# Advaith-Sajeev/LiDAR-Vision-VQA

Measured on AMD Instinct MI355X. Metric: fused tokens/sec/GPU + cross-attn MFMA-roofline % (32k pts x 196 patches), higher is better.
Workload: dtype bf16; 1 GPU; BASELINE configs[1]: 32768-pt scenes (Dist-C) -> hard voxelise (0.1, 0.1, 0.2) T=10 max=60000 + MeanVFE; pillars (0.2, 0.2, 8.0) T=20 max=30000 -> PillarVFE[64] -> PointPillarScatter 512x512 (as an index map; sparse key stream: K|V computed only for the cells with a pillar in their 3x3 neighbourhood, by LayerNorm and the K|V projection folded onto the 64-channel conv token, every other key from th; parallelism=scene-parallel x1

## Files before the change

### include/lvq.h

```cpp
#ifndef LVQ_H
#define LVQ_H

#include <stddef.h>
#include <stdint.h>

#ifdef __cplusplus
extern "C" {
#endif

typedef void *lvq_stream_t;
typedef uint16_t lvq_bf16;

enum {
    LVQ_OK = 0,
    LVQ_EINVAL = -1,
    LVQ_EWORKSPACE = -2,
    LVQ_ELAUNCH = -3,
    LVQ_EOVERFLOW = -4,
    LVQ_EUNSUPPORTED = -5
};

const char *lvq_version(void);
const char *lvq_strerror(int code);

typedef struct lvq_tuning {
    int32_t attn_no32;
    int32_t attn32_nw;
    int32_t attn_pipe;
    int32_t attn_nsplit;
    int32_t attn_qt;
    int32_t attn_nw;
    int32_t gemm_no_gemv;
    int32_t gemm_stream_c_mb;
    int32_t gemm_no256;
    int32_t gemm_no256x256;
    int32_t gemm_256x256_min_tiles;
    int32_t gemm_ln_tiles;
    int32_t pillar_vfe_generic;
    int32_t voxel_path;
    int32_t pairs_one_wg;
    int32_t ca_fused_variant;
    uint64_t ca_fused_stamps;
    int32_t reserved[8];
} lvq_tuning;
void lvq_tuning_defaults(lvq_tuning *t);
int lvq_set_tuning(const lvq_tuning *t);
int lvq_get_tuning(lvq_tuning *t);


int lvq_mask_points_by_range(const float *pts, int64_t n, int c, const float *range_host, uint8_t *keep,
                             lvq_stream_t stream);

size_t lvq_voxelize_hard_workspace_bytes(int64_t n_points, int n_scenes);
int lvq_voxelize_hard(const float *pts, const int32_t *scene_off, int64_t n_points, int n_scenes, int c,
                      const float *range_host, const float *vsize_host, const int32_t *grid_host,
                      int max_pts, int max_voxels, int break_on_cap, int64_t voxel_capacity,
                      float *voxels, int32_t *coords_bzyx, int32_t *num_pts, int32_t *scene_voxel_off,
                      void *ws, size_t ws_bytes, lvq_stream_t stream);

int lvq_voxelize_mean(const float *pts, const int32_t *scene_off, int64_t n_points, int n_scenes, int c,
                      const float *range_host, const float *vsize_host, const int32_t *grid_host, int max_pts,
                      int max_voxels, int64_t voxel_capacity, float *voxel_features, int32_t *coords_bzyx,
                      int32_t *num_pts, int32_t *scene_voxel_off, void *ws, size_t ws_bytes, lvq_stream_t stream);

int lvq_mean_vfe(const float *voxels, const int32_t *num_pts, int64_t m_cap, const int32_t *n_voxels_dev,
                 int t, int c, float *out, lvq_stream_t stream);

int lvq_pillar_vfe(const float *voxels, const int32_t *num_pts, const int32_t *coords_bzyx, int64_t m_cap,
                   const int32_t *n_voxels_dev, int t, int c, int n_layers, const float *const *w_host,
                   const float *const *scale_host, const float *const *shift_host, const int32_t *cin_host,
                   const int32_t *cout_host, int flags, const float *vsize_host, const float *offset_host,
                   float *out, lvq_stream_t stream);

size_t lvq_voxelize_dynamic_workspace_bytes(int64_t n_points, int batch_size, const int32_t *grid_host, int ndim);
int lvq_voxelize_dynamic(const float *pts, int64_t n, int c, int batch_size, const float *range_host,
                         const float *vsize_host, const int32_t *grid_host, int ndim, int32_t *unq_inv,
// ... 215 lines not shown
```

### lidar-vision-vqa_amd/_ffi.py

```python
from __future__ import annotations

import ctypes
import os
import re
from typing import List, Optional, Sequence

import torch

_HERE = os.path.dirname(os.path.abspath(__file__))
LIB_PATH = os.environ.get("LVQ_LIB_PATH") or os.path.join(_HERE, "liblvq_hip.so")
HEADER_PATH = os.path.join(os.path.dirname(_HERE), "include", "lvq.h")

LVQ_OK = 0
LVQ_EUNSUPPORTED = -5


class LvqError(RuntimeError):
    pass


_lib: Optional[ctypes.CDLL] = None


class Tuning(ctypes.Structure):
    _fields_ = [(n, ctypes.c_int32) for n in (
        "attn_no32", "attn32_nw", "attn_pipe", "attn_nsplit", "attn_qt", "attn_nw", "gemm_no_gemv", "gemm_stream_c_mb", "gemm_no256",
        "gemm_no256x256", "gemm_256x256_min_tiles", "gemm_ln_tiles", "pillar_vfe_generic", "voxel_path", "pairs_one_wg",
        "ca_fused_variant")] + [("ca_fused_stamps", ctypes.c_uint64), ("reserved", ctypes.c_int32 * 8)]


TUNING_FIELDS = tuple(n for n, _ in Tuning._fields_ if n != "reserved")


def tuning_from_env(env=None) -> dict:
    e = os.environ if env is None else env

    def flag(name):
        return 1 if e.get(name) else 0

    def num(name):
        return int(e[name]) if e.get(name) else 0

    return {
        "attn_no32": flag("LVQ_ATTN_NO32"), "attn32_nw": num("LVQ_ATTN32_NW"),
        "attn_pipe": -1 if e.get("LVQ_ATTN_NO_PIPE") else flag("LVQ_ATTN_PIPE"),
        "attn_nsplit": num("LVQ_ATTN_NSPLIT"), "attn_qt": num("LVQ_ATTN_QT"), "attn_nw": num("LVQ_ATTN_NW"),
        "gemm_no_gemv": flag("LVQ_GEMM_NO_GEMV"),
        "gemm_stream_c_mb": -1 if e.get("LVQ_GEMM_NO_STREAM_C") else num("LVQ_GEMM_STREAM_C_MB"),
        "gemm_no256": flag("LVQ_GEMM_NO256"), "gemm_no256x256": flag("LVQ_GEMM_NO256X256"),
        "gemm_256x256_min_tiles": num("LVQ_GEMM_256X256_MIN_TILES"), "gemm_ln_tiles": flag("LVQ_GEMM_LN_TILES"),
        "pillar_vfe_generic": flag("LVQ_PILLAR_VFE_GENERIC"),
        "voxel_path": 2 if e.get("LVQ_VOXEL_LEGACY") else flag("LVQ_VOXEL_BINNED"),
        "pairs_one_wg": flag("LVQ_PAIRS_ONE_WG"), "ca_fused_variant": num("LVQ_CA_DBG"), "ca_fused_stamps": 0,
    }


def set_tuning(**fields) -> dict:
    rec = tuning_from_env()
    for k, v in fields.items():
        if k not in TUNING_FIELDS:
            raise LvqError(f"lvq_tuning has no field {k!r}")
        rec[k] = int(v)
    t = Tuning()
    for k, v in rec.items():
        setattr(t, k, v)
    check(lib().lvq_set_tuning(ctypes.byref(t)), "lvq_set_tuning")
    return rec


def get_tuning() -> dict:
    t = Tuning()
    check(lib().lvq_get_tuning(ctypes.byref(t)), "lvq_get_tuning")
    return {k: int(getattr(t, k)) for k in TUNING_FIELDS}


class tuning:

    def __init__(self, **fields):
        self.fields = fields

    def __enter__(self):
        self.old = get_tuning()
        cur = dict(self.old)
        cur.update({k: int(v) for k, v in self.fields.items()})
        _push(cur)
        return self
# ... 87 lines not shown
```

### lidar-vision-vqa_amd/csrc/bev_tiles.hip

```cpp
#include "common.h"
#include <type_traits>
#include <utility>

namespace bt {

typedef __attribute__((ext_vector_type(8))) short bf16x8;
typedef __attribute__((ext_vector_type(4))) float f32x4;
typedef __attribute__((ext_vector_type(2))) __bf16 bf16x2_t;
typedef uint32_t u32x4 __attribute__((ext_vector_type(4)));

__device__ __forceinline__ uint32_t pack_bf16(float a, float b) {
    bf16x2_t p = {(__bf16)a, (__bf16)b};
    return *reinterpret_cast<uint32_t *>(&p);
}
typedef _Float16 f16x2_t __attribute__((ext_vector_type(2)));
__device__ __forceinline__ uint32_t pack_f16(float a, float b) {
    f16x2_t p = {(_Float16)a, (_Float16)b};
    return __builtin_bit_cast(uint32_t, p);
}

constexpr int TS = 8, TCELLS = 64;
constexpr int NPIECE = 8, PCELLS = 8;
constexpr int PH = 4, PW = 6, PHALO = PH * PW;
constexpr int NSLOT = NPIECE * PHALO;
// ... 782 lines not shown
            };
            f32x4 te_a[2 * JH], te_b[2 * JH];
            int2 pd_a, pd_b;
            request(0, te_a, pd_a);
            if (has_nx) conv_tile(ih_nx, buf ^ 1);
            request(1, te_b, pd_b);
            emit(0, te_a, pd_a);
            request(2, te_a, pd_a);
            emit(1, te_b, pd_b);
            request(3, te_b, pd_b);
            emit(2, te_a, pd_a);
            emit(3, te_b, pd_b);
        }
        buf ^= 1;
    }
}

struct ConvArgs {
    const float *feat;
    const int32_t *idx;
    const int32_t *live_list;
    const int2 *piece_dirty;
    const int32_t *counts;
    const float *w9, *b9;
    const uint16_t *rh, *rl;
    const float *r0;
    float c0, inv_d, eps;
    int S, H, W;
    uint16_t *th, *tl;
    float *rstd;
    int32_t *key;
};

template <bool X3>
__global__ void __launch_bounds__(512) k_conv_rows(ConvArgs a) {
    constexpr int C = 64, NWV = 8;
    extern __shared__ __attribute__((aligned(16))) uint8_t smem[];
    uint16_t *t_hi = reinterpret_cast<uint16_t *>(smem);
    uint16_t *t_lo = t_hi + 2 * TCELLS * C;
    float *halo = reinterpret_cast<float *>(t_lo + 2 * TCELLS * C);
    int32_t *idxh = reinterpret_cast<int32_t *>(halo + NSLOT * C);
    float *part = reinterpret_cast<float *>(idxh + 2 * 256);
    float *w9s = part + 2 * 4 * TCELLS;
    float *b9s = w9s + 9 * C;
    float *r0s = b9s + C;
    uint16_t *r_hi = reinterpret_cast<uint16_t *>(r0s + C);
    uint16_t *r_lo = r_hi + C * C;
    const int tid = threadIdx.x, lane = tid & 63, wid = tid >> 6, l15 = lane & 15, g4 = lane >> 4;
    const int tw = a.W / TS;
    const int n_live = a.counts[0];
    const int64_t n_groups = ((int64_t)n_live + NPIECE - 1) / NPIECE;
    const int64_t g_begin = blockIdx.x, g_end = n_groups, g_step = gridDim.x;

    for (int e = tid; e < 9 * C; e += 512) w9s[e] = a.w9[(e % C) * 9 + e / C];
    if (tid < C) { b9s[tid] = a.b9 ? a.b9[tid] : 0.f; r0s[tid] = a.r0[tid]; }
    for (int e = tid; e < C * C / 8; e += 512) {
        reinterpret_cast<u32x4 *>(r_hi)[e] = reinterpret_cast<const u32x4 *>(a.rh)[e];
        if (X3) reinterpret_cast<u32x4 *>(r_lo)[e] = reinterpret_cast<const u32x4 *>(a.rl)[e];
    }
    auto load_idx = [&](int64_t g, int &code_out) -> int {
        code_out = -1;
        if (tid >= NSLOT) return -1;
        const int j = tid / PHALO, hc = tid - j * PHALO;
        const int64_t k = g * NPIECE + j;
        if (k >= n_live) return -1;
        const int code = a.live_list[k];
        code_out = code;
        const int p = code & 7, ts = code >> 3, t = ts / a.S, sc = ts - t * a.S;
        int y0, x0;
        piece_origin(t, p, tw, y0, x0);
        const int gy = y0 - 1 + hc / PW, gx = x0 - 1 + hc % PW;
        return (gy >= 0 && gy < a.H && gx >= 0 && gx < a.W) ? a.idx[((int64_t)sc * a.H + gy) * a.W + gx] : -1;
    };
    auto store_idx = [&](int32_t *ih, int v, int code) {
        if (tid < NSLOT) {
            ih[tid] = v;
            if (tid % PHALO == 0) ih[200 + tid / PHALO] = code;
        }
    };
    auto dma_halo = [&](const int32_t *ih) {
        for (int q = wid; q < NSLOT / 4; q += NWV) {
            const int slot = q * 4 + (lane >> 4);
            const int row = ih[slot];
            if (row >= 0)
                __builtin_amdgcn_global_load_lds((const __attribute__((address_space(1))) void *)(a.feat + (int64_t)row * C + 4 * l15),
                                                 (__attribute__((address_space(3))) void *)(halo + q * 4 * C), 16, 0, 0);
        }
    };
    auto conv_tile = [&](const int32_t *ih, int buf, int64_t g) {
        const int cell = tid >> 3, cg = (tid & 7) * 8, hb = (cell >> 3) * PHALO, cy = (cell >> 2) & 1, cx = cell & 3;
        float acc[8];
#pragma unroll
        for (int c = 0; c < 8; ++c) acc[c] = b9s[cg + c];
#pragma unroll
        for (int rr = 0; rr < 3; ++rr)
#pragma unroll
            for (int k = 0; k < 3; ++k) {
                const int slot = hb + (cy + rr) * PW + cx + k;
                if (ih[slot] >= 0) {
                    const f32x4 v0 = *reinterpret_cast<const f32x4 *>(halo + slot * C + cg), v1 = *reinterpret_cast<const f32x4 *>(halo + slot * C + cg + 4);
                    const f32x4 k0 = *reinterpret_cast<const f32x4 *>(w9s + (rr * 3 + k) * C + cg), k1 = *reinterpret_cast<const f32x4 *>(w9s + (rr * 3 + k) * C + cg + 4);
#pragma unroll
                    for (int c = 0; c < 4; ++c) { acc[c] = fmaf(v0[c], k0[c], acc[c]); acc[4 + c] = fmaf(v1[c], k1[c], acc[4 + c]); }
                }
            }
        uint32_t hi[4], lo[4];
#pragma unroll
        for (int c = 0; c < 4; ++c) {
            const float y0 = gelu_erf(acc[2 * c]), y1 = gelu_erf(acc[2 * c + 1]);
            hi[c] = pack_bf16(y0, y1);
            lo[c] = pack_bf16(y0 - __uint_as_float(hi[c] << 16), y1 - __uint_as_float(hi[c] & 0xffff0000u));
        }
        const int ch = (tid & 7) ^ ((cell >> 1) & 7);
        *reinterpret_cast<u32x4 *>(t_hi + (buf * TCELLS + cell) * C + ch * 8) = u32x4{hi[0], hi[1], hi[2], hi[3]};
        if (X3) *reinterpret_cast<u32x4 *>(t_lo + (buf * TCELLS + cell) * C + ch * 8) = u32x4{lo[0], lo[1], lo[2], lo[3]};
        const int code = ih[200 + (cell >> 3)];
        if (code >= 0) {
            const int2 pd = a.piece_dirty[g * NPIECE + (cell >> 3)];
            if ((pd.y >> (cell & 7)) & 1) {
                const int64_t orow = pd.x + __popc((unsigned)pd.y & ((1u << (cell & 7)) - 1u));
                *reinterpret_cast<u32x4 *>(a.th + orow * C + cg) = u32x4{hi[0], hi[1], hi[2], hi[3]};
                if (X3) *reinterpret_cast<u32x4 *>(a.tl + orow * C + cg) = u32x4{lo[0], lo[1], lo[2], lo[3]};
            }
        }
    };
    auto load_t = [&](int buf, int gq, bf16x8 &th0, bf16x8 &th1, bf16x8 &tl0, bf16x8 &tl1) {
        const int row = gq * 16 + l15;
        const int c0 = (g4 ^ ((row >> 1) & 7)) * 8, c1 = ((4 + g4) ^ ((row >> 1) & 7)) * 8;
        th0 = *reinterpret_cast<const bf16x8 *>(t_hi + (buf * TCELLS + row) * C + c0);
        th1 = *reinterpret_cast<const bf16x8 *>(t_hi + (buf * TCELLS + row) * C + c1);
        if (X3) {
            tl0 = *reinterpret_cast<const bf16x8 *>(t_lo + (buf * TCELLS + row) * C + c0);
            tl1 = *reinterpret_cast<const bf16x8 *>(t_lo + (buf * TCELLS + row) * C + c1);
        }
    };

    if (tid < 256) { idxh[tid] = -1; idxh[256 + tid] = -1; }
    __syncthreads();
    if (g_begin >= g_end) return;
    {
        int c0, c1;
        const int i0 = load_idx(g_begin, c0);
        const int i1 = g_begin + g_step < g_end ? load_idx(g_begin + g_step, c1) : (c1 = -1, -1);
        store_idx(idxh, i0, c0);
        store_idx(idxh + 256, i1, c1);
    }
    __syncthreads();
    dma_halo(idxh);
    asm volatile("s_waitcnt vmcnt(0)" ::: "memory");
    __syncthreads();
    conv_tile(idxh, 0, g_begin);
    int buf = 0;
    for (int64_t g = g_begin, it = 0; g < g_end; g += g_step, ++it) {
        __syncthreads();
        const int32_t *ih_cur = idxh + (it & 1) * 256, *ih_nx = idxh + ((it + 1) & 1) * 256;
        const bool has_nx = g + g_step < g_end, has_n2 = g + 2 * g_step < g_end;
        if (has_nx) dma_halo(ih_nx);
        const int my_code = tid < TCELLS ? ih_cur[200 + (tid >> 3)] : -1;
        int c2 = -1;
        const int i2 = has_n2 ? load_idx(g + 2 * g_step, c2) : -1;
        {
            const int rt = wid & 3;
            const uint16_t *rp = r_hi + (16 * rt + l15) * C + 8 * g4, *rpl = r_lo + (16 * rt + l15) * C + 8 * g4;
            const bf16x8 ra0 = *reinterpret_cast<const bf16x8 *>(rp), ra1 = *reinterpret_cast<const bf16x8 *>(rp + 32);
            bf16x8 rl0 = ra0, rl1 = ra1;
            if (X3) { rl0 = *reinterpret_cast<const bf16x8 *>(rpl); rl1 = *reinterpret_cast<const bf16x8 *>(rpl + 32); }
            const f32x4 rinit = *reinterpret_cast<const f32x4 *>(r0s + 16 * rt + 4 * g4);
#pragma unroll
            for (int u = 0; u < 2; ++u) {
                const int gq = 2 * (wid >> 2) + u;
                bf16x8 th0, th1, tl0, tl1;
                load_t(buf, gq, th0, th1, tl0, tl1);
                f32x4 v = rinit;
                v = __builtin_amdgcn_mfma_f32_16x16x32_bf16(ra0, th0, v, 0, 0, 0);
                v = __builtin_amdgcn_mfma_f32_16x16x32_bf16(ra1, th1, v, 0, 0, 0);
                if (X3) {
                    v = __builtin_amdgcn_mfma_f32_16x16x32_bf16(ra0, tl0, v, 0, 0, 0);
                    v = __builtin_amdgcn_mfma_f32_16x16x32_bf16(ra1, tl1, v, 0, 0, 0);
                    v = __builtin_amdgcn_mfma_f32_16x16x32_bf16(rl0, th0, v, 0, 0, 0);
                    v = __builtin_amdgcn_mfma_f32_16x16x32_bf16(rl1, th1, v, 0, 0, 0);
                }
                float sq = (v[0] * v[0] + v[1] * v[1]) + (v[2] * v[2] + v[3] * v[3]);
                sq += __shfl_xor(sq, 16);
                sq += __shfl_xor(sq, 32);
                if (g4 == 0) part[(buf * 4 + rt) * TCELLS + gq * 16 + l15] = sq;
            }
        }
        asm volatile("s_waitcnt vmcnt(0)" ::: "memory");
        __syncthreads();
        store_idx(idxh + (it & 1) * 256, i2, c2);
        if (tid < TCELLS && my_code >= 0) {
            const int cell = tid;
            const int2 pd = a.piece_dirty[g * NPIECE + (cell >> 3)];
            if ((pd.y >> (cell & 7)) & 1) {
                const int64_t orow = pd.x + __popc((unsigned)pd.y & ((1u << (cell & 7)) - 1u));
                const float *pr = part + buf * 4 * TCELLS;
                const float ss = (pr[cell] + pr[TCELLS + cell]) + (pr[2 * TCELLS + cell] + pr[3 * TCELLS + cell]) + a.c0;
                a.rstd[orow] = 1.0f / sqrtf(ss * a.inv_d + a.eps);
                a.key[orow] = ((my_code >> 3) / a.S) * TCELLS + (my_code & 7) * PCELLS + (cell & 7);
            }
        }
        if (has_nx) conv_tile(ih_nx, buf ^ 1, g + g_step);
        buf ^= 1;
    }
}

struct KvRowArgs {
    const uint16_t *th, *tl;
    const float *rstd;
    const int32_t *key;
    const int32_t *n_rows;
    const uint16_t *mh, *ml;
    const float *m0;
    const float *te;
    uint16_t *out;
    int k_fp16;
};

template <int N> __device__ __forceinline__ void vm_wait() { asm volatile("s_waitcnt vmcnt(%0)" ::"n"(N) : "memory"); }
template <int OFF> __device__ __forceinline__ void vm_load16(f32x4 &d, const void *p) {
    asm volatile("global_load_dwordx4 %0, %1, off offset:%2" : "=&v"(d) : "v"(p), "n"(OFF) : "memory");
}
template <class T> __device__ __forceinline__ void vm_load4(T &d, const void *p) {
    static_assert(sizeof(T) == 4, "one dword");
    asm volatile("global_load_dword %0, %1, off" : "=&v"(d) : "v"(p) : "memory");
}
__device__ __forceinline__ void vm_dma16(const void *src, uint32_t dst) {
    uint32_t keep;
    asm volatile("s_mov_b32 %0, m0\n\ts_mov_b32 m0, %2\n\ts_nop 0\n\tglobal_load_lds_dwordx4 %1, off\n\ts_mov_b32 m0, %0"
                 : "=&s"(keep) : "v"(src), "s"(dst) : "memory");
}
template <class T> __device__ __forceinline__ void landed(T &x) { asm volatile("" : "+v"(x)); }
template <int... I, class F> __device__ __forceinline__ void static_for(std::integer_sequence<int, I...>, F &&f) { (f(std::integral_constant<int, I>{}), ...); }
template <int N, class F> __device__ __forceinline__ void static_for(F &&f) { static_for(std::make_integer_sequence<int, N>{}, f); }

template <int J, bool X3, bool TH>
__global__ void __launch_bounds__(512) k_kv_rows(KvRowArgs a) {
    constexpr int N = 128 * J, C = 64, JH = J / 2;
    static_assert(J % 2 == 0, "even J");
    extern __shared__ __attribute__((aligned(16))) uint8_t smem[];
    uint16_t *t_hi = reinterpret_cast<uint16_t *>(smem);
    uint16_t *t_lo = t_hi + 2 * TCELLS * C;
    float *pbias = reinterpret_cast<float *>(t_lo + 2 * TCELLS * C);
    constexpr int SROW = N + 8;
    uint16_t *sbuf = reinterpret_cast<uint16_t *>(pbias + N);
    const int tid = threadIdx.x, lane = tid & 63, wid = tid >> 6, l15 = lane & 15, g4 = lane >> 4;
    const int64_t n_rows = *a.n_rows;
    const int64_t n_groups = (n_rows + TCELLS - 1) / TCELLS;
    const bool x8 = gridDim.x >= 16 && gridDim.x % 16 == 0;
    const int nxcd = x8 ? 8 : 1;
    const int xcd = x8 ? (int)blockIdx.x & 7 : 0;
    const int half = x8 ? ((int)blockIdx.x >> 3) & 1 : (int)blockIdx.x & 1;
    const int wg_r = x8 ? (int)blockIdx.x >> 4 : (int)blockIdx.x >> 1, wg_R = x8 ? (int)gridDim.x >> 4 : ((int)gridDim.x + 1) >> 1;
    const int64_t per_x = (n_groups + nxcd - 1) / nxcd;
    const int64_t x_begin = (int64_t)xcd * per_x, x_end = x_begin + per_x < n_groups ? x_begin + per_x : n_groups;
    const int64_t g_begin = x_begin + wg_r, g_end = x_end, g_step = wg_R;
    const int ncol0 = half * N;
    const bool as_f16 = a.k_fp16 != 0 && half == 0;
    for (int e = tid; e < N; e += 512) pbias[e] = a.m0[ncol0 + e];

    bf16x8 wf[J][2], wfl[X3 ? J : 1][2];
#pragma unroll
    for (int j = 0; j < J; ++j) {
        const int n = ncol0 + 16 * J * wid + (TH ? 32 * (j >> 1) + 8 * (l15 >> 2) + 4 * (j & 1) + (l15 & 3) : 16 * j + l15);
        wf[j][0] = *reinterpret_cast<const bf16x8 *>(a.mh + (int64_t)n * C + 8 * g4);
        wf[j][1] = *reinterpret_cast<const bf16x8 *>(a.mh + (int64_t)n * C + 32 + 8 * g4);
        if (X3) {
// ... 233 lines not shown
}

extern "C" int lvq_bev_tile_kv(const float *pillar_feat, const int32_t *idx_map, const int32_t *live_list, const int32_t *piece_dirty,
                               const int32_t *counts, int64_t cap_tiles, int batch, int ny, int nx, int c_in, const float *w9, const float *b9,
                               const lvq_bf16 *m, const lvq_bf16 *m_lo, const float *m0, const lvq_bf16 *r, const lvq_bf16 *r_lo, const float *r0,
                               float c0, int d_ln, float eps, const void *t_tiled, int t_f16, int n, int k_fp16, lvq_bf16 *kv, void *ws,
                               size_t ws_bytes, lvq_stream_t stream) {
    if (batch <= 0 || ny <= 0 || nx <= 0 || cap_tiles <= 0 || d_ln <= 0 || !idx_map || !live_list || !piece_dirty || !counts || !w9 || !m || !m0 || !r ||
        !r0 || !t_tiled || !kv)
        return LVQ_EINVAL;
    if ((m_lo == nullptr) != (r_lo == nullptr)) return LVQ_EINVAL;
    if ((k_fp16 || t_f16) && ws == nullptr) return LVQ_EUNSUPPORTED;
    if (c_in != 64 || (ny % 8) || (nx % 8) || (n % 256) || n < 256 || n > 1024) return LVQ_EUNSUPPORTED;
    if (((uintptr_t)pillar_feat | (uintptr_t)m | (uintptr_t)m_lo | (uintptr_t)r | (uintptr_t)r_lo | (uintptr_t)m0 | (uintptr_t)r0 | (uintptr_t)t_tiled |
         (uintptr_t)kv) & 15)
        return LVQ_EUNSUPPORTED;
    bt::KvArgs a;
    a.feat = pillar_feat; a.idx = idx_map; a.live_list = live_list; a.piece_dirty = reinterpret_cast<const int2 *>(piece_dirty); a.counts = counts;
    a.w9 = w9; a.b9 = b9; a.mh = m; a.ml = m_lo; a.m0 = m0; a.rh = r; a.rl = r_lo; a.r0 = r0; a.c0 = c0; a.inv_d = 1.0f / (float)d_ln; a.eps = eps;
    a.te = static_cast<const float *>(t_tiled); a.S = batch; a.H = ny; a.W = nx; a.out = kv;
    hipStream_t st = lvq_s(stream);
    const bool x3 = m_lo != nullptr;
    if (ws != nullptr) {
        LvqArena arena(ws, ws_bytes);
        uint16_t *th = arena.take<uint16_t>((size_t)cap_tiles * 64 * 64);
        uint16_t *tl = arena.take<uint16_t>((size_t)cap_tiles * 64 * 64);
        float *rstd = arena.take<float>((size_t)cap_tiles * 64);
        int32_t *key = arena.take<int32_t>((size_t)cap_tiles * 64);
        if (!arena.ok) return LVQ_EWORKSPACE;
        bt::ConvArgs c;
        c.feat = pillar_feat; c.idx = idx_map; c.live_list = live_list; c.piece_dirty = a.piece_dirty; c.counts = counts; c.w9 = w9; c.b9 = b9;
        c.rh = r; c.rl = r_lo; c.r0 = r0; c.c0 = c0; c.inv_d = a.inv_d; c.eps = eps; c.S = batch; c.H = ny; c.W = nx;
        c.th = th; c.tl = x3 ? tl : nullptr; c.rstd = rstd; c.key = key;
        const size_t lds = (size_t)2 * 2 * bt::TCELLS * 64 * 2 + (size_t)bt::NSLOT * 64 * 4 + 2 * 256 * 4 + (size_t)2 * 4 * bt::TCELLS * 4 + 9 * 64 * 4 +
                           64 * 4 + 64 * 4 + (size_t)2 * 64 * 64 * 2;
        static LvqLdsOnce once;
        if (!lvq_ensure_lds(once, {(const void *)bt::k_conv_rows<false>, (const void *)bt::k_conv_rows<true>}, lds)) return LVQ_ELAUNCH;
        int64_t grid = (int64_t)lvq_cu_count();
        if (grid > cap_tiles) grid = cap_tiles;
        if (x3) hipLaunchKernelGGL((bt::k_conv_rows<true>), dim3((unsigned)grid), dim3(512), lds, st, c);
        else    hipLaunchKernelGGL((bt::k_conv_rows<false>), dim3((unsigned)grid), dim3(512), lds, st, c);
        bt::KvRowArgs k;
        k.th = th; k.tl = x3 ? tl : nullptr; k.rstd = rstd; k.key = key; k.n_rows = counts + 2; k.mh = m; k.ml = m_lo; k.m0 = m0; k.te = static_cast<const float *>(t_tiled); k.out = kv; k.k_fp16 = k_fp16;
        switch (n / 128) {
            case 2: return launch_kv_rows<2>(k, x3, t_f16 != 0, cap_tiles, st);
            case 4: return launch_kv_rows<4>(k, x3, t_f16 != 0, cap_tiles, st);
            case 6: return launch_kv_rows<6>(k, x3, t_f16 != 0, cap_tiles, st);
            case 8: return launch_kv_rows<8>(k, x3, t_f16 != 0, cap_tiles, st);
            default: return LVQ_EUNSUPPORTED;
        }
    }
    switch (n / 128) {
        case 2: return launch_tile_kv<2>(a, x3, cap_tiles, st);
        case 4: return launch_tile_kv<4>(a, x3, cap_tiles, st);
        case 6: return launch_tile_kv<6>(a, x3, cap_tiles, st);
        case 8: return launch_tile_kv<8>(a, x3, cap_tiles, st);
        default: return LVQ_EUNSUPPORTED;
    }
}

extern "C" int lvq_bev_scene_pairs(const int32_t *row_src, int batch, int n_tiles, int row_base, int cap_tiles, int32_t *pair_src,
                                   int32_t *pair_info, lvq_stream_t stream) {
    if (!row_src || !pair_src || !pair_info || batch <= 0 || n_tiles <= 0 || cap_tiles <= 0 || row_base < 0) return LVQ_EINVAL;
    if (((uintptr_t)row_src & 15) || (int64_t)n_tiles * bt::TCELLS > 0x7fffffff || batch > 65535) return LVQ_EUNSUPPORTED;
    if (cap_tiles >= n_tiles && cap_tiles >= 2 && !lvq_tune().pairs_one_wg) {
        const int64_t ne = (int64_t)n_tiles * bt::TCELLS;
        int64_t chunk = (ne + 63) / 64;
        chunk = (chunk + 1023) / 1024 * 1024;
        const int nch = (int)((ne + chunk - 1) / chunk);
        hipLaunchKernelGGL(bt::k_scene_pair_count, dim3(nch, batch), dim3(bt::PAIR2_NT), 0, lvq_s(stream), row_src, n_tiles, row_base, cap_tiles, (int)chunk,
                           pair_src);
        hipLaunchKernelGGL(bt::k_scene_pair_write, dim3(nch, batch), dim3(bt::PAIR2_NT), 0, lvq_s(stream), row_src, n_tiles, row_base, cap_tiles, (int)chunk,
// ... 47 lines not shown
```

### lidar-vision-vqa_amd/fusion.py

```python
from __future__ import annotations

import math
import os
from typing import Dict, List, Optional, Tuple

import torch
import torch.nn as nn

from . import _ffi as F
from . import autograd_route as AG
from . import ops
from .ops import BF

NUM_VIEWS = 6
CAM_VIEWS = ("CAM_FRONT", "CAM_FRONT_RIGHT", "CAM_FRONT_LEFT", "CAM_BACK", "CAM_BACK_RIGHT", "CAM_BACK_LEFT")


class _HipModule(nn.Module):

    def __init__(self):
        super().__init__()
        object.__setattr__(self, "_wcache", {})
        self.precision: Optional[str] = None

# ... 362 lines not shown
        ver = tuple((p.data_ptr(), p._version) for p in params) + (self._mode(), fused, k16, bool(os.environ.get("LVQ_KV_ONE_LAUNCH")),
                                                                   bool(os.environ.get("LVQ_KV_T_FP16")))
        key = ("kv_buffer", H, W, dev)
        hw, d = H * W, self.d_model
        rows = hw + batch * hw
        hit = self._pe_cache.get(key)
        if hit is not None and hit[0] == ver:
            if hit[1][0].shape[0] >= rows:
                return hit[1]
            bufs = []
            for old in hit[1]:
                buf = torch.empty((rows, 2 * d), dtype=torch.bfloat16, device=dev)
                buf[:hw].copy_(old[:hw])
                bufs.append(buf)
            self._pe_cache[key] = (ver, bufs)
            return bufs
        self._pe_cache.pop(("signed_totals", H, W, dev), None)
        idx = torch.full((1, H, W), -1, dtype=torch.int32, device=dev)
        live, dirty, src, counts = ops.bev_tiles(idx, 1, H, W, dev, 0, force_all=True)
        feat = torch.zeros((1, C), dtype=torch.float32, device=dev)
        x = None if fused else self._tile_tokens(feat, idx, live, dirty, counts, hw, 1, H, W)
        bufs = []
        for li, blk in enumerate(self.blocks):
            blk.precision = self.precision
            buf = torch.empty((rows, 2 * d), dtype=torch.bfloat16, device=dev)
            if fused:
                self._tile_kv(li, feat, idx, live, dirty, counts, hw, 1, H, W, buf[:hw], k_fp16=k16 and li == 0)
            else:
                ops.linear_live_rows(x, blk._w(blk.ca.in_proj_weight), blk.ca.in_proj_bias, counts[2:], (d, 3 * d), out=buf[:hw])
            bufs.append(buf)
        self._pe_cache[key] = (ver, bufs)
        return bufs

    def _q16_ok(self, blk: "VATBlock", qp: BF) -> bool:
        params = [self.query, self.view_embed, blk.sa_ln.weight, blk.sa_ln.bias, blk.sa.in_proj_weight, blk.sa.in_proj_bias, blk.sa.out_proj.weight,
                  blk.sa.out_proj.bias, blk.ca_ln.weight, blk.ca_ln.bias, blk.ca.in_proj_weight, blk.ca.in_proj_bias]
        ver = tuple((p.data_ptr(), p._version) for p in params) + (self._mode(),)
        hit = self._pe_cache.get("q16_ok")
        if hit is not None and hit[0] == ver:
            return hit[1]
        dh = blk.d_model // blk.n_heads
        qmax = float(ops.to_f32(qp).abs().max()) * (1.0 / math.sqrt(dh)) * 1.4426950408889634
        ok = qmax < 3.0e4
        self._pe_cache["q16_ok"] = (ver, ok)
        return ok

    STREAM_GUARD_MAX = 0.5

    def stream_guard(self, C: int, H: int, W: int, dev) -> float:
        blk = self.blocks[0]
        params = [self.query, self.view_embed, blk.sa_ln.weight, blk.sa_ln.bias, blk.sa.in_proj_weight, blk.sa.in_proj_bias, blk.sa.out_proj.weight,
                  blk.sa.out_proj.bias, blk.ca_ln.weight, blk.ca_ln.bias, blk.ca.in_proj_weight, blk.ca.in_proj_bias,
                  self.refine[0].weight, self.refine[0].bias, self.proj.weight, self.proj.bias, self.norm_tokens.weight, self.norm_tokens.bias,
                  self.geo_mlp[0].weight, self.geo_mlp[0].bias, self.geo_mlp[2].weight, self.geo_mlp[2].bias]
        ver = tuple((p.data_ptr(), p._version) for p in params)
        key = ("stream_guard", H, W, dev)
        hit = self._pe_cache.get(key)
        if hit is not None and hit[0] == ver:
            return hit[1]
        keep = self.precision
        try:
            self.precision = "mixed"
            blk.precision = "mixed"
            _, qp = blk.shared_query_side(self._queries(1), self.n_queries)
            table = self._kv_buffers(C, H, W, dev, 1, False)[0]
            dh = blk.d_model // blk.n_heads
            g = float(ops.stream_guard(qp[0], table[:H * W], blk.n_heads, 1.0 / math.sqrt(dh)).max())
        finally:
            self.precision = keep
            blk.precision = keep
        self._pe_cache[key] = (ver, g)
        return g

    def guard_counters(self) -> Tuple[int, int, float]:
        st = getattr(self, "_guard_stats", None)
        if st is None:
            return (0, 0, 0.0)
        a, b, c, _ = st.cpu().tolist()
        return int(a), int(b), float(torch.tensor([c], dtype=torch.int32).view(torch.float32))

    def _audit_scene(self, qp_hi: torch.Tensor, table: torch.Tensor, src: torch.Tensor, scene: int, n_keys: int, k16: bool = False) -> torch.Tensor:
        blk = self.blocks[0]
        d = blk.d_model
        rows = src.view(-1, n_keys)[scene].long()
        k_scene = table[:, :d].index_select(0, rows)
        if k16:
            k_scene = k_scene.view(torch.float16).to(torch.bfloat16)
        return ops.stream_guard(qp_hi, k_scene, blk.n_heads, 1.0 / math.sqrt(d // blk.n_heads)).max()

    def _audit(self, qps: List[torch.Tensor], kvs: List[torch.Tensor], src: torch.Tensor, scenes, n_keys: int, k16: bool) -> torch.Tensor:
        nq = self.n_queries
        g = [self._audit_scene(q if q.shape[0] == nq else q[b * nq:(b + 1) * nq], kvs[li], src, b, n_keys, k16 and li == 0)
             for li, q in enumerate(qps) for b in scenes]
        return torch.stack(g).max()

    def _guard_poll(self) -> bool:
        pend = getattr(self, "_guard_pending", None)
# ... 28 lines not shown
        return tot

    def forward_pillars(self, pillar_features: torch.Tensor, coords_bzyx: torch.Tensor, n_live: Optional[torch.Tensor],
                        batch: int, H: int, W: int, all_tiles_live: bool = False) -> torch.Tensor:
        self._guard(pillar_features)
        C = pillar_features.shape[1]
        dev = pillar_features.device
        feat = _f32(pillar_features)
        tiled = self._sparse_route_ok(C, H, W)
        guarded = tiled and self._mode() in ("mixed", "mixed16") and not os.environ.get("LVQ_NO_STREAM_GUARD")
        if guarded:
            ver = self._guard_version()
            if getattr(self, "_guard_ver", None) != ver:
                object.__setattr__(self, "_guard_ver", ver)
                object.__setattr__(self, "_guard_calls", 0)
                object.__setattr__(self, "_guard_pending", None)
            tripped = getattr(self, "_guard_tripped", None) == ver
            if not tripped and self._guard_poll():
                object.__setattr__(self, "_guard_tripped", ver)
                tripped = True
            if tripped or self.stream_guard(C, H, W, dev) > self.STREAM_GUARD_MAX:
                return self._forward_pillars_hilo(pillar_features, coords_bzyx, n_live, batch, H, W, all_tiles_live)
        if not tiled:
            t = ops.pillar_dwconv3x3_gelu(feat, coords_bzyx, n_live, batch, H, W,
                                          self.refine[0].weight.detach().reshape(C, 9).contiguous(), self.refine[0].bias, self._split())
            return self._decode(self._tokens_to_model(t, H, W, dev), batch, H, W)
        nt = (H // 8) * (W // 8)
        fused = not os.environ.get("LVQ_NO_FUSED_KV")
        signed = not all_tiles_live and not os.environ.get("LVQ_NO_SIGNED_STREAM")
        q2_1 = qp = None
        k16 = False
        if signed:
            self.blocks[0].precision = self.precision
            q2_1, qp = self.blocks[0].shared_query_side(self._queries(1), self.n_queries)
            k16 = (self._mode() == "mixed16" and fused and self._kv_fold(C, H, W, dev)[4] < 3.0e4 and self._q16_ok(self.blocks[0], qp))
        kvs = self._kv_buffers(C, H, W, dev, batch, k16)
        idx = ops.pillar_index_map(coords_bzyx, n_live, batch, H, W)
        live, dirty, src, counts = ops.bev_tiles(idx, batch, H, W, dev, H * W, force_all=all_tiles_live)
        x_live = None if fused else self._tile_tokens(feat, idx, live, dirty, counts, batch * nt * 64, batch, H, W)
        q2 = None if signed else self._queries(batch)
        qps = []
        for li, (blk, table) in enumerate(zip(self.blocks, kvs)):
            blk.precision = self.precision
            if fused:
                self._tile_kv(li, feat, idx, live, dirty, counts, batch * nt * 64, batch, H, W, table[H * W:], k_fp16=k16 and li == 0)
            if li == 0 and signed:
                totals = self._signed_totals(blk, qp, table, H, W, dev, k_fp16=k16)
                if getattr(self, "_guard_stats", None) is None or self._guard_stats.device != dev:
                    object.__setattr__(self, "_guard_stats", torch.zeros(4, dtype=torch.int32, device=dev))
                q2 = blk.forward_tokens_tiled_signed(q2_1, qp, totals, x_live, table, src, counts[2:], batch, self.n_queries, nt, k_fp16=k16,
                                                     stats=self._guard_stats)
                qps.append(qp[0])
            else:
                q2, qp_l = blk.forward_tokens_tiled(q2, x_live, table, src, counts[2:], batch, self.n_queries, nt)
                qps.append(qp_l[0])
        self._last_tile_counts = counts
        if guarded:
            calls = self._guard_calls
            object.__setattr__(self, "_guard_calls", calls + 1)
            if self.strict_parity or calls == 0:
                g = self._audit(qps, kvs, src, range(batch), H * W, k16)
                if float(g) > self.STREAM_GUARD_MAX:
                    object.__setattr__(self, "_guard_tripped", self._guard_version())
                    return self._forward_pillars_hilo(pillar_features, coords_bzyx, n_live, batch, H, W, all_tiles_live)
            elif self.audit_every and calls % self.audit_every == 0:
                self._guard_submit(self._audit(qps, kvs, src, [(calls // self.audit_every) % batch], H * W, k16))
        return _post_head(self, q2, self.final_ln, self.post).view(batch, self.n_queries, self.d_model)
# ... 172 lines not shown
```

Baseline: 972,000 fused tokens/s.

## Re-pipeline conv-rows kernel with register weights and cache the query-side projection

The k_conv_rows kernel now keeps the depthwise weights, bias and the 64x64 R matrix in registers instead of staging them in LDS. It double-buffers the halo rather than the conv tile, and prefetches live-list codes and dirty masks through an 8-deep LDS ring using inline-asm loads and async LDS DMA, so index and metadata fetches overlap the conv and MFMA work. Separately, the shared query-side projection, which depends only on parameters, is cached per parameter version instead of being recomputed on every forward call. A tuning hook for the conv grid size is added; the trade-off is higher register pressure and more fragile hand-written waitcnt and barrier ordering.

```diff
diff --git a/include/lvq.h b/include/lvq.h
--- a/include/lvq.h
+++ b/include/lvq.h
@@ -41,7 +41,8 @@
     int32_t pairs_one_wg;
     int32_t ca_fused_variant;
     uint64_t ca_fused_stamps;
-    int32_t reserved[8];
+    int32_t conv_rows_grid;
+    int32_t reserved[7];
 } lvq_tuning;
 void lvq_tuning_defaults(lvq_tuning *t);
 int lvq_set_tuning(const lvq_tuning *t);
diff --git a/lidar-vision-vqa_amd/_ffi.py b/lidar-vision-vqa_amd/_ffi.py
--- a/lidar-vision-vqa_amd/_ffi.py
+++ b/lidar-vision-vqa_amd/_ffi.py
@@ -26,7 +26,7 @@
     _fields_ = [(n, ctypes.c_int32) for n in (
         "attn_no32", "attn32_nw", "attn_pipe", "attn_nsplit", "attn_qt", "attn_nw", "gemm_no_gemv", "gemm_stream_c_mb", "gemm_no256",
         "gemm_no256x256", "gemm_256x256_min_tiles", "gemm_ln_tiles", "pillar_vfe_generic", "voxel_path", "pairs_one_wg",
-        "ca_fused_variant")] + [("ca_fused_stamps", ctypes.c_uint64), ("reserved", ctypes.c_int32 * 8)]
+        "ca_fused_variant")] + [("ca_fused_stamps", ctypes.c_uint64), ("conv_rows_grid", ctypes.c_int32), ("reserved", ctypes.c_int32 * 7)]
 
 
 TUNING_FIELDS = tuple(n for n, _ in Tuning._fields_ if n != "reserved")
@@ -52,6 +52,7 @@
         "pillar_vfe_generic": flag("LVQ_PILLAR_VFE_GENERIC"),
         "voxel_path": 2 if e.get("LVQ_VOXEL_LEGACY") else flag("LVQ_VOXEL_BINNED"),
         "pairs_one_wg": flag("LVQ_PAIRS_ONE_WG"), "ca_fused_variant": num("LVQ_CA_DBG"), "ca_fused_stamps": 0,
+        "conv_rows_grid": 0,
     }
 
 
diff --git a/lidar-vision-vqa_amd/csrc/bev_tiles.hip b/lidar-vision-vqa_amd/csrc/bev_tiles.hip
--- a/lidar-vision-vqa_amd/csrc/bev_tiles.hip
+++ b/lidar-vision-vqa_amd/csrc/bev_tiles.hip
@@ -838,76 +838,114 @@
     int32_t *key;
 };
 
+typedef int i32x2 __attribute__((ext_vector_type(2)));
+template <int N> __device__ __forceinline__ void vm_wait() { asm volatile("s_waitcnt vmcnt(%0)" ::"n"(N) : "memory"); }
+template <int OFF> __device__ __forceinline__ void vm_load16(f32x4 &d, const void *p) {
+    asm volatile("global_load_dwordx4 %0, %1, off offset:%2" : "=&v"(d) : "v"(p), "n"(OFF) : "memory");
+}
+__device__ __forceinline__ void vm_load8(i32x2 &d, const void *p) { asm volatile("global_load_dwordx2 %0, %1, off" : "=&v"(d) : "v"(p) : "memory"); }
+template <class T> __device__ __forceinline__ void vm_load4(T &d, const void *p) {
+    static_assert(sizeof(T) == 4, "one dword");
+    asm volatile("global_load_dword %0, %1, off" : "=&v"(d) : "v"(p) : "memory");
+}
+__device__ __forceinline__ void vm_dma16(const void *src, uint32_t dst) {
+    uint32_t keep;
+    asm volatile("s_mov_b32 %0, m0\n\ts_mov_b32 m0, %2\n\ts_nop 0\n\tglobal_load_lds_dwordx4 %1, off\n\ts_mov_b32 m0, %0"
+                 : "=&s"(keep) : "v"(src), "s"(dst) : "memory");
+}
+template <class T> __device__ __forceinline__ void landed(T &x) { asm volatile("" : "+v"(x)); }
+template <int... I, class F> __device__ __forceinline__ void static_for(std::integer_sequence<int, I...>, F &&f) { (f(std::integral_constant<int, I>{}), ...); }
+template <int N, class F> __device__ __forceinline__ void static_for(F &&f) { static_for(std::make_integer_sequence<int, N>{}, f); }
+__device__ __forceinline__ void lds_barrier() {
+    asm volatile("s_waitcnt lgkmcnt(0)" ::: "memory");
+    __builtin_amdgcn_s_barrier();
+    asm volatile("" ::: "memory");
+}
+
 template <bool X3>
 __global__ void __launch_bounds__(512) k_conv_rows(ConvArgs a) {
-    constexpr int C = 64, NWV = 8;
+    constexpr int C = 64, NWV = 8, RING = 8;
     extern __shared__ __attribute__((aligned(16))) uint8_t smem[];
     uint16_t *t_hi = reinterpret_cast<uint16_t *>(smem);
-    uint16_t *t_lo = t_hi + 2 * TCELLS * C;
-    float *halo = reinterpret_cast<float *>(t_lo + 2 * TCELLS * C);
-    int32_t *idxh = reinterpret_cast<int32_t *>(halo + NSLOT * C);
-    float *part = reinterpret_cast<float *>(idxh + 2 * 256);
-    float *w9s = part + 2 * 4 * TCELLS;
-    float *b9s = w9s + 9 * C;
-    float *r0s = b9s + C;
-    uint16_t *r_hi = reinterpret_cast<uint16_t *>(r0s + C);
-    uint16_t *r_lo = r_hi + C * C;
+    uint16_t *t_lo = t_hi + TCELLS * C;
+    float *halo = reinterpret_cast<float *>(t_lo + TCELLS * C);
+    int32_t *idxh = reinterpret_cast<int32_t *>(halo + 2 * NSLOT * C);
+    int32_t *mcode = idxh + 2 * 256;
+    i32x2 *mdirty = reinterpret_cast<i32x2 *>(mcode + RING * NPIECE);
+    float *part = reinterpret_cast<float *>(mdirty + RING * NPIECE);
     const int tid = threadIdx.x, lane = tid & 63, wid = tid >> 6, l15 = lane & 15, g4 = lane >> 4;
     const int tw = a.W / TS;
     const int n_live = a.counts[0];
     const int64_t n_groups = ((int64_t)n_live + NPIECE - 1) / NPIECE;
-    const int64_t g_begin = blockIdx.x, g_end = n_groups, g_step = gridDim.x;
-
-    for (int e = tid; e < 9 * C; e += 512) w9s[e] = a.w9[(e % C) * 9 + e / C];
-    if (tid < C) { b9s[tid] = a.b9 ? a.b9[tid] : 0.f; r0s[tid] = a.r0[tid]; }
-    for (int e = tid; e < C * C / 8; e += 512) {
-        reinterpret_cast<u32x4 *>(r_hi)[e] = reinterpret_cast<const u32x4 *>(a.rh)[e];
-        if (X3) reinterpret_cast<u32x4 *>(r_lo)[e] = reinterpret_cast<const u32x4 *>(a.rl)[e];
-    }
-    auto load_idx = [&](int64_t g, int &code_out) -> int {
-        code_out = -1;
-        if (tid >= NSLOT) return -1;
+    const int64_t g_begin = blockIdx.x, g_step = gridDim.x;
+    if (g_begin >= n_groups) return;
+    const int n_my = (int)((n_groups - g_begin + g_step - 1) / g_step);
+
+    float wk[9][8], bk[8];
+#pragma unroll
+    for (int c = 0; c < 8; ++c) {
+        const int ch = (tid & 7) * 8 + c;
+        bk[c] = a.b9 ? a.b9[ch] : 0.f;
+#pragma unroll
+        for (int k = 0; k < 9; ++k) wk[k][c] = a.w9[ch * 9 + k];
+    }
+    const int rt = wid & 3;
+    bf16x8 ra0, ra1, rl0, rl1;
+    {
+        const uint16_t *rp = a.rh + (16 * rt + l15) * C + 8 * g4;
+        ra0 = *reinterpret_cast<const bf16x8 *>(rp);
+        ra1 = *reinterpret_cast<const bf16x8 *>(rp + 32);
+        rl0 = ra0; rl1 = ra1;
+        if (X3) {
+            const uint16_t *rpl = a.rl + (16 * rt + l15) * C + 8 * g4;
+            rl0 = *reinterpret_cast<const bf16x8 *>(rpl);
+            rl1 = *reinterpret_cast<const bf16x8 *>(rpl + 32);
+        }
+    }
+    f32x4 rinit = *reinterpret_cast<const f32x4 *>(a.r0 + 16 * rt + 4 * g4);
+
+    auto piece_k = [&](int o, int j, bool &ok) -> int64_t {
+        const int64_t grp = g_begin + (int64_t)o * g_step, k = grp * NPIECE + j;
+        ok = o < n_my && k < n_live;
+        return ok ? k : 0;
+    };
+    auto idx_off = [&](int o, bool &ok) -> int64_t {
+        ok = false;
+        if (tid >= NSLOT) return 0;
         const int j = tid / PHALO, hc = tid - j * PHALO;
-        const int64_t k = g * NPIECE + j;
-        if (k >= n_live) return -1;
-        const int code = a.live_list[k];
-        code_out = code;
+        const int code = mcode[(o & (RING - 1)) * NPIECE + j];
+        if (code < 0) return 0;
         const int p = code & 7, ts = code >> 3, t = ts / a.S, sc = ts - t * a.S;
         int y0, x0;
         piece_origin(t, p, tw, y0, x0);
         const int gy = y0 - 1 + hc / PW, gx = x0 - 1 + hc % PW;
-        return (gy >= 0 && gy < a.H && gx >= 0 && gx < a.W) ? a.idx[((int64_t)sc * a.H + gy) * a.W + gx] : -1;
-    };
-    auto store_idx = [&](int32_t *ih, int v, int code) {
-        if (tid < NSLOT) {
-            ih[tid] = v;
-            if (tid % PHALO == 0) ih[200 + tid / PHALO] = code;
-        }
-    };
-    auto dma_halo = [&](const int32_t *ih) {
+        if (gy < 0 || gy >= a.H || gx < 0 || gx >= a.W) return 0;
+        ok = true;
+        return ((int64_t)sc * a.H + gy) * a.W + gx;
+    };
+    const uint32_t lds_halo = (uint32_t)(uintptr_t)((__attribute__((address_space(3))) float *)halo);
+    auto dma_halo = [&](const int32_t *ih, int hbuf) {
         for (int q = wid; q < NSLOT / 4; q += NWV) {
-            const int slot = q * 4 + (lane >> 4);
-            const int row = ih[slot];
-            if (row >= 0)
-                __builtin_amdgcn_global_load_lds((const __attribute__((address_space(1))) void *)(a.feat + (int64_t)row * C + 4 * l15),
-                                                 (__attribute__((address_space(3))) void *)(halo + q * 4 * C), 16, 0, 0);
-        }
-    };
-    auto conv_tile = [&](const int32_t *ih, int buf, int64_t g) {
+            const int row = ih[q * 4 + (lane >> 4)];
+            const uint32_t dst = __builtin_amdgcn_readfirstlane(lds_halo + (uint32_t)((hbuf * NSLOT + q * 4) * C * 4));
+            if (row >= 0) vm_dma16(a.feat + (int64_t)row * C + 4 * l15, dst);
+        }
+    };
+    auto conv_tile = [&](const int32_t *ih, const float *hl, int o) {
         const int cell = tid >> 3, cg = (tid & 7) * 8, hb = (cell >> 3) * PHALO, cy = (cell >> 2) & 1, cx = cell & 3;
         float acc[8];
 #pragma unroll
-        for (int c = 0; c < 8; ++c) acc[c] = b9s[cg + c];
+        for (int c = 0; c < 8; ++c) acc[c] = bk[c];
 #pragma unroll
         for (int rr = 0; rr < 3; ++rr)
 #pragma unroll
             for (int k = 0; k < 3; ++k) {
                 const int slot = hb + (cy + rr) * PW + cx + k;
                 if (ih[slot] >= 0) {
-                    const f32x4 v0 = *reinterpret_cast<const f32x4 *>(halo + slot * C + cg), v1 = *reinterpret_cast<const f32x4 *>(halo + slot * C + cg + 4);
-                    const f32x4 k0 = *reinterpret_cast<const f32x4 *>(w9s + (rr * 3 + k) * C + cg), k1 = *reinterpret_cast<const f32x4 *>(w9s + (rr * 3 + k) * C + cg + 4);
-#pragma unroll
-                    for (int c = 0; c < 4; ++c) { acc[c] = fmaf(v0[c], k0[c], acc[c]); acc[4 + c] = fmaf(v1[c], k1[c], acc[4 + c]); }
+                    const f32x4 v0 = *reinterpret_cast<const f32x4 *>(hl + slot * C + cg), v1 = *reinterpret_cast<const f32x4 *>(hl + slot * C + cg + 4);
+                    const float *kk = wk[rr * 3 + k];
+#pragma unroll
+                    for (int c = 0; c < 4; ++c) { acc[c] = fmaf(v0[c], kk[c], acc[c]); acc[4 + c] = fmaf(v1[c], kk[4 + c], acc[4 + c]); }
                 }
             }
         uint32_t hi[4], lo[4];
@@ -918,11 +956,11 @@
             lo[c] = pack_bf16(y0 - __uint_as_float(hi[c] << 16), y1 - __uint_as_float(hi[c] & 0xffff0000u));
         }
         const int ch = (tid & 7) ^ ((cell >> 1) & 7);
-        *reinterpret_cast<u32x4 *>(t_hi + (buf * TCELLS + cell) * C + ch * 8) = u32x4{hi[0], hi[1], hi[2], hi[3]};
-        if (X3) *reinterpret_cast<u32x4 *>(t_lo + (buf * TCELLS + cell) * C + ch * 8) = u32x4{lo[0], lo[1], lo[2], lo[3]};
-        const int code = ih[200 + (cell >> 3)];
-        if (code >= 0) {
-            const int2 pd = a.piece_dirty[g * NPIECE + (cell >> 3)];
+        *reinterpret_cast<u32x4 *>(t_hi + cell * C + ch * 8) = u32x4{hi[0], hi[1], hi[2], hi[3]};
+        if (X3) *reinterpret_cast<u32x4 *>(t_lo + cell * C + ch * 8) = u32x4{lo[0], lo[1], lo[2], lo[3]};
+        const int m = (o & (RING - 1)) * NPIECE + (cell >> 3);
+        if (mcode[m] >= 0) {
+            const i32x2 pd = mdirty[m];
             if ((pd.y >> (cell & 7)) & 1) {
                 const int64_t orow = pd.x + __popc((unsigned)pd.y & ((1u << (cell & 7)) - 1u));
                 *reinterpret_cast<u32x4 *>(a.th + orow * C + cg) = u32x4{hi[0], hi[1], hi[2], hi[3]};
@@ -930,84 +968,100 @@
             }
         }
     };
-    auto load_t = [&](int buf, int gq, bf16x8 &th0, bf16x8 &th1, bf16x8 &tl0, bf16x8 &tl1) {
-        const int row = gq * 16 + l15;
-        const int c0 = (g4 ^ ((row >> 1) & 7)) * 8, c1 = ((4 + g4) ^ ((row >> 1) & 7)) * 8;
-        th0 = *reinterpret_cast<const bf16x8 *>(t_hi + (buf * TCELLS + row) * C + c0);
-        th1 = *reinterpret_cast<const bf16x8 *>(t_hi + (buf * TCELLS + row) * C + c1);
-        if (X3) {
-            tl0 = *reinterpret_cast<const bf16x8 *>(t_lo + (buf * TCELLS + row) * C + c0);
-            tl1 = *reinterpret_cast<const bf16x8 *>(t_lo + (buf * TCELLS + row) * C + c1);
-        }
-    };
-
-    if (tid < 256) { idxh[tid] = -1; idxh[256 + tid] = -1; }
+    auto row_sums = [&]() {
+#pragma unroll
+        for (int u = 0; u < 2; ++u) {
+            const int gq = 2 * (wid >> 2) + u;
+            const int row = gq * 16 + l15;
+            const int c0 = (g4 ^ ((row >> 1) & 7)) * 8, c1 = ((4 + g4) ^ ((row >> 1) & 7)) * 8;
+            const bf16x8 th0 = *reinterpret_cast<const bf16x8 *>(t_hi + row * C + c0), th1 = *reinterpret_cast<const bf16x8 *>(t_hi + row * C + c1);
+            f32x4 v = rinit;
+            v = __builtin_amdgcn_mfma_f32_16x16x32_bf16(ra0, th0, v, 0, 0, 0);
+            v = __builtin_amdgcn_mfma_f32_16x16x32_bf16(ra1, th1, v, 0, 0, 0);
+            if (X3) {
+                const bf16x8 tl0 = *reinterpret_cast<const bf16x8 *>(t_lo + row * C + c0), tl1 = *reinterpret_cast<const bf16x8 *>(t_lo + row * C + c1);
+                v = __builtin_amdgcn_mfma_f32_16x16x32_bf16(ra0, tl0, v, 0, 0, 0);
+                v = __builtin_amdgcn_mfma_f32_16x16x32_bf16(ra1, tl1, v, 0, 0, 0);
+                v = __builtin_amdgcn_mfma_f32_16x16x32_bf16(rl0, th0, v, 0, 0, 0);
+                v = __builtin_amdgcn_mfma_f32_16x16x32_bf16(rl1, th1, v, 0, 0, 0);
+            }
+            float sq = (v[0] * v[0] + v[1] * v[1]) + (v[2] * v[2] + v[3] * v[3]);
+            sq += __shfl_xor(sq, 16);
+            sq += __shfl_xor(sq, 32);
+            if (g4 == 0) part[rt * TCELLS + gq * 16 + l15] = sq;
+        }
+    };
+    auto finish_rows = [&](int o) {
+        if (wid != NWV - 1) return;
+        const int cell = lane, m = (o & (RING - 1)) * NPIECE + (cell >> 3);
+        const int code = mcode[m];
+        if (code < 0) return;
+        const i32x2 pd = mdirty[m];
+        if ((pd.y >> (cell & 7)) & 1) {
+            const int64_t orow = pd.x + __popc((unsigned)pd.y & ((1u << (cell & 7)) - 1u));
+            const float ss = (part[cell] + part[TCELLS + cell]) + (part[2 * TCELLS + cell] + part[3 * TCELLS + cell]) + a.c0;
+            a.rstd[orow] = 1.0f / sqrtf(ss * a.inv_d + a.eps);
+            a.key[orow] = ((code >> 3) / a.S) * TCELLS + (code & 7) * PCELLS + (cell & 7);
+        }
+    };
+
+    if (tid < 4 * NPIECE) {
+        bool ok;
+        const int64_t k = piece_k(tid >> 3, tid & 7, ok);
+        const int code = a.live_list[k];
+        const int2 pd = a.piece_dirty[k];
+        mcode[tid] = ok ? code : -1;
+        mdirty[tid] = ok ? i32x2{pd.x, pd.y} : i32x2{0, 0};
+    }
     __syncthreads();
-    if (g_begin >= g_end) return;
     {
-        int c0, c1;
-        const int i0 = load_idx(g_begin, c0);
-        const int i1 = g_begin + g_step < g_end ? load_idx(g_begin + g_step, c1) : (c1 = -1, -1);
-        store_idx(idxh, i0, c0);
-        store_idx(idxh + 256, i1, c1);
-    }
-    __syncthreads();
-    dma_halo(idxh);
-    asm volatile("s_waitcnt vmcnt(0)" ::: "memory");
-    __syncthreads();
-    conv_tile(idxh, 0, g_begin);
-    int buf = 0;
-    for (int64_t g = g_begin, it = 0; g < g_end; g += g_step, ++it) {
+        bool k0, k1, k2;
+        const int64_t o0 = idx_off(0, k0), o1 = idx_off(1, k1), o2 = idx_off(2, k2);
+        const int i0 = a.idx[o0], i1 = a.idx[o1], i2 = a.idx[o2];
+        if (tid < 256) { idxh[tid] = k0 ? i0 : -1; idxh[256 + tid] = k1 ? i1 : -1; }
         __syncthreads();
-        const int32_t *ih_cur = idxh + (it & 1) * 256, *ih_nx = idxh + ((it + 1) & 1) * 256;
-        const bool has_nx = g + g_step < g_end, has_n2 = g + 2 * g_step < g_end;
-        if (has_nx) dma_halo(ih_nx);
-        const int my_code = tid < TCELLS ? ih_cur[200 + (tid >> 3)] : -1;
-        int c2 = -1;
-        const int i2 = has_n2 ? load_idx(g + 2 * g_step, c2) : -1;
-        {
-            const int rt = wid & 3;
-            const uint16_t *rp = r_hi + (16 * rt + l15) * C + 8 * g4, *rpl = r_lo + (16 * rt + l15) * C + 8 * g4;
-            const bf16x8 ra0 = *reinterpret_cast<const bf16x8 *>(rp), ra1 = *reinterpret_cast<const bf16x8 *>(rp + 32);
-            bf16x8 rl0 = ra0, rl1 = ra1;
-            if (X3) { rl0 = *reinterpret_cast<const bf16x8 *>(rpl); rl1 = *reinterpret_cast<const bf16x8 *>(rpl + 32); }
-            const f32x4 rinit = *reinterpret_cast<const f32x4 *>(r0s + 16 * rt + 4 * g4);
-#pragma unroll
-            for (int u = 0; u < 2; ++u) {
-                const int gq = 2 * (wid >> 2) + u;
-                bf16x8 th0, th1, tl0, tl1;
-                load_t(buf, gq, th0, th1, tl0, tl1);
-                f32x4 v = rinit;
-                v = __builtin_amdgcn_mfma_f32_16x16x32_bf16(ra0, th0, v, 0, 0, 0);
-                v = __builtin_amdgcn_mfma_f32_16x16x32_bf16(ra1, th1, v, 0, 0, 0);
-                if (X3) {
-                    v = __builtin_amdgcn_mfma_f32_16x16x32_bf16(ra0, tl0, v, 0, 0, 0);
-                    v = __builtin_amdgcn_mfma_f32_16x16x32_bf16(ra1, tl1, v, 0, 0, 0);
-                    v = __builtin_amdgcn_mfma_f32_16x16x32_bf16(rl0, th0, v, 0, 0, 0);
-                    v = __builtin_amdgcn_mfma_f32_16x16x32_bf16(rl1, th1, v, 0, 0, 0);
-                }
-                float sq = (v[0] * v[0] + v[1] * v[1]) + (v[2] * v[2] + v[3] * v[3]);
-                sq += __shfl_xor(sq, 16);
-                sq += __shfl_xor(sq, 32);
-                if (g4 == 0) part[(buf * 4 + rt) * TCELLS + gq * 16 + l15] = sq;
-            }
-        }
-        asm volatile("s_waitcnt vmcnt(0)" ::: "memory");
+        dma_halo(idxh, 0);
+        dma_halo(idxh + 256, 1);
+        vm_wait<0>();
+        landed(ra0); landed(ra1); landed(rl0); landed(rl1); landed(rinit);
+#pragma unroll
+        for (int c = 0; c < 8; ++c) {
+            landed(bk[c]);
+#pragma unroll
+            for (int k = 0; k < 9; ++k) landed(wk[k][c]);
+        }
         __syncthreads();
-        store_idx(idxh + (it & 1) * 256, i2, c2);
-        if (tid < TCELLS && my_code >= 0) {
-            const int cell = tid;
-            const int2 pd = a.piece_dirty[g * NPIECE + (cell >> 3)];
-            if ((pd.y >> (cell & 7)) & 1) {
-                const int64_t orow = pd.x + __popc((unsigned)pd.y & ((1u << (cell & 7)) - 1u));
-                const float *pr = part + buf * 4 * TCELLS;
-                const float ss = (pr[cell] + pr[TCELLS + cell]) + (pr[2 * TCELLS + cell] + pr[3 * TCELLS + cell]) + a.c0;
-                a.rstd[orow] = 1.0f / sqrtf(ss * a.inv_d + a.eps);
-                a.key[orow] = ((my_code >> 3) / a.S) * TCELLS + (my_code & 7) * PCELLS + (cell & 7);
-            }
-        }
-        if (has_nx) conv_tile(ih_nx, buf ^ 1, g + g_step);
-        buf ^= 1;
+        conv_tile(idxh, halo, 0);
+        __syncthreads();
+        row_sums();
+        if (tid < 256) idxh[tid] = k2 ? i2 : -1;
+        __syncthreads();
+    }
+    for (int it = 0; it < n_my; ++it) {
+        const int cur = it & 1, nx = cur ^ 1;
+        const bool has_nx = it + 1 < n_my;
+        dma_halo(idxh + cur * 256, cur);
+        bool ok_i, ok_m;
+        const int64_t off_i = idx_off(it + 3, ok_i);
+        const int64_t k_m = piece_k(it + 4, tid & 7, ok_m);
+        int iw, mc;
+        i32x2 md;
+        vm_load4(iw, a.idx + off_i);
+        vm_load4(mc, a.live_list + k_m);
+        vm_load8(md, a.piece_dirty + k_m);
+        finish_rows(it);
+        if (has_nx) conv_tile(idxh + nx * 256, halo + nx * NSLOT * C, it + 1);
+        lds_barrier();
+        if (has_nx) row_sums();
+        vm_wait<0>();
+        landed(iw); landed(mc); landed(md);
+        if (tid < 256) idxh[nx * 256 + tid] = ok_i ? iw : -1;
+        if (tid < NPIECE) {
+            const int m = ((it + 4) & (RING - 1)) * NPIECE + tid;
+            mcode[m] = ok_m ? mc : -1;
+            mdirty[m] = ok_m ? md : i32x2{0, 0};
+        }
+        lds_barrier();
     }
 }
 
@@ -1022,23 +1076,6 @@
     uint16_t *out;
     int k_fp16;
 };
-
-template <int N> __device__ __forceinline__ void vm_wait() { asm volatile("s_waitcnt vmcnt(%0)" ::"n"(N) : "memory"); }
-template <int OFF> __device__ __forceinline__ void vm_load16(f32x4 &d, const void *p) {
-    asm volatile("global_load_dwordx4 %0, %1, off offset:%2" : "=&v"(d) : "v"(p), "n"(OFF) : "memory");
-}
-template <class T> __device__ __forceinline__ void vm_load4(T &d, const void *p) {
-    static_assert(sizeof(T) == 4, "one dword");
-    asm volatile("global_load_dword %0, %1, off" : "=&v"(d) : "v"(p) : "memory");
-}
-__device__ __forceinline__ void vm_dma16(const void *src, uint32_t dst) {
-    uint32_t keep;
-    asm volatile("s_mov_b32 %0, m0\n\ts_mov_b32 m0, %2\n\ts_nop 0\n\tglobal_load_lds_dwordx4 %1, off\n\ts_mov_b32 m0, %0"
-                 : "=&s"(keep) : "v"(src), "s"(dst) : "memory");
-}
-template <class T> __device__ __forceinline__ void landed(T &x) { asm volatile("" : "+v"(x)); }
-template <int... I, class F> __device__ __forceinline__ void static_for(std::integer_sequence<int, I...>, F &&f) { (f(std::integral_constant<int, I>{}), ...); }
-template <int N, class F> __device__ __forceinline__ void static_for(F &&f) { static_for(std::make_integer_sequence<int, N>{}, f); }
 
 template <int J, bool X3, bool TH>
 __global__ void __launch_bounds__(512) k_kv_rows(KvRowArgs a) {
@@ -1338,12 +1375,14 @@
         c.feat = pillar_feat; c.idx = idx_map; c.live_list = live_list; c.piece_dirty = a.piece_dirty; c.counts = counts; c.w9 = w9; c.b9 = b9;
         c.rh = r; c.rl = r_lo; c.r0 = r0; c.c0 = c0; c.inv_d = a.inv_d; c.eps = eps; c.S = batch; c.H = ny; c.W = nx;
         c.th = th; c.tl = x3 ? tl : nullptr; c.rstd = rstd; c.key = key;
-        const size_t lds = (size_t)2 * 2 * bt::TCELLS * 64 * 2 + (size_t)bt::NSLOT * 64 * 4 + 2 * 256 * 4 + (size_t)2 * 4 * bt::TCELLS * 4 + 9 * 64 * 4 +
-                           64 * 4 + 64 * 4 + (size_t)2 * 64 * 64 * 2;
+        const size_t lds = (size_t)2 * bt::TCELLS * 64 * 2 + (size_t)2 * bt::NSLOT * 64 * 4 + 2 * 256 * 4 + (size_t)8 * bt::NPIECE * (4 + 8) +
+                           (size_t)4 * bt::TCELLS * 4;
         static LvqLdsOnce once;
         if (!lvq_ensure_lds(once, {(const void *)bt::k_conv_rows<false>, (const void *)bt::k_conv_rows<true>}, lds)) return LVQ_ELAUNCH;
         int64_t grid = (int64_t)lvq_cu_count();
-        if (grid > cap_tiles) grid = cap_tiles;
+        const int hook = lvq_tune().conv_rows_grid;
+        if (hook > 0) grid = hook < grid ? hook : grid;
+        else if (grid > cap_tiles) grid = cap_tiles;
         if (x3) hipLaunchKernelGGL((bt::k_conv_rows<true>), dim3((unsigned)grid), dim3(512), lds, st, c);
         else    hipLaunchKernelGGL((bt::k_conv_rows<false>), dim3((unsigned)grid), dim3(512), lds, st, c);
         bt::KvRowArgs k;
diff --git a/lidar-vision-vqa_amd/fusion.py b/lidar-vision-vqa_amd/fusion.py
--- a/lidar-vision-vqa_amd/fusion.py
+++ b/lidar-vision-vqa_amd/fusion.py
@@ -418,6 +418,18 @@
         self._pe_cache[key] = (ver, bufs)
         return bufs
 
+    def _query_side(self, blk: "VATBlock", dev) -> Tuple[torch.Tensor, BF]:
+        params = [self.query, self.view_embed, blk.sa_ln.weight, blk.sa_ln.bias, blk.sa.in_proj_weight, blk.sa.in_proj_bias, blk.sa.out_proj.weight,
+                  blk.sa.out_proj.bias, blk.ca_ln.weight, blk.ca_ln.bias, blk.ca.in_proj_weight, blk.ca.in_proj_bias]
+        ver = tuple((p.data_ptr(), p._version) for p in params)
+        key = ("query_side", blk._mode(), dev)
+        hit = self._pe_cache.get(key)
+        if hit is not None and hit[0] == ver:
+            return hit[1]
+        pair = blk.shared_query_side(self._queries(1), self.n_queries)
+        self._pe_cache[key] = (ver, pair)
+        return pair
+
     def _q16_ok(self, blk: "VATBlock", qp: BF) -> bool:
         params = [self.query, self.view_embed, blk.sa_ln.weight, blk.sa_ln.bias, blk.sa.in_proj_weight, blk.sa.in_proj_bias, blk.sa.out_proj.weight,
                   blk.sa.out_proj.bias, blk.ca_ln.weight, blk.ca_ln.bias, blk.ca.in_proj_weight, blk.ca.in_proj_bias]
@@ -448,7 +460,7 @@
         try:
             self.precision = "mixed"
             blk.precision = "mixed"
-            _, qp = blk.shared_query_side(self._queries(1), self.n_queries)
+            _, qp = self._query_side(blk, dev)
             table = self._kv_buffers(C, H, W, dev, 1, False)[0]
             dh = blk.d_model // blk.n_heads
             g = float(ops.stream_guard(qp[0], table[:H * W], blk.n_heads, 1.0 / math.sqrt(dh)).max())
@@ -543,7 +555,7 @@
         k16 = False
         if signed:
             self.blocks[0].precision = self.precision
-            q2_1, qp = self.blocks[0].shared_query_side(self._queries(1), self.n_queries)
+            q2_1, qp = self._query_side(self.blocks[0], dev)
             k16 = (self._mode() == "mixed16" and fused and self._kv_fold(C, H, W, dev)[4] < 3.0e4 and self._q16_ok(self.blocks[0], qp))
         kvs = self._kv_buffers(C, H, W, dev, batch, k16)
         idx = ops.pillar_index_map(coords_bzyx, n_live, batch, H, W)
```

After: 990,900 fused tokens/s, median of 6. 1.02x the previous value.
